# menonsamir/spiral

Hardware: AMD Instinct MI355X
Metric: server ms/query + DB GB/s vs HBM roofline, 2^20 x 256B (lower is better)
Workload: dtype u32 residues, 32x32->64-bit integer MAC (two 28-bit CRT primes)

## Files before the change

### spiral_amd/csrc/host_common.h

```cpp
#pragma once
#include <hip/hip_runtime.h>

#include <algorithm>
#include <atomic>
#include <cstdarg>
#include <cstdio>
#include <cstdlib>
#include <cstring>
#include <string>
#include <vector>

#include "../../include/spiral_gpu.h"
#include "common.h"
#include "kernels.h"
#include "seed_device.h"
#include "transform_jobs.h"

namespace spiral {
namespace host {

extern thread_local std::string g_err;
extern std::atomic<uint64_t> g_pack_lane_batches;
extern std::atomic<uint64_t> g_db_export_ns;

// ... 112 lines not shown
    std::vector<void*> ptrs;
    ~Scratch() {
        for (void* p : ptrs) (void)hipFree(p);
    }
    uint64_t* get(size_t words) {
        void* p = nullptr;
        if (hipMalloc(&p, (words ? words : 1) * sizeof(uint64_t)) != hipSuccess) return nullptr;
        ptrs.push_back(p);
        return (uint64_t*)p;
    }
    uint64_t* upload(const uint64_t* host, size_t words) {
        uint64_t* d = get(words);
        if (d && hipMemcpy(d, host, words * sizeof(uint64_t), hipMemcpyHostToDevice) != hipSuccess) return nullptr;
        return d;
    }
};

inline int current_tables(DeviceTables* t) {
    int dev = 0;
    HIP_OK(hipGetDevice(&dev));
    if (tables_get(dev, t) != 0) return fail("twiddle table setup failed on device %d", dev);
    return 0;
}

struct ExpandWork {
    uint64_t* raw;
    uint64_t* g;
};
inline size_t expand_g_polys(uint32_t g, uint32_t t_exp, uint32_t t_exp_right) {
    size_t half = (size_t)1 << (g ? g - 1 : 0);
    return half * ((size_t)t_exp + 1 + t_exp_right + 1);
}

struct ExpandShard {
    uint32_t rank, g_log, j_log;
};

inline void run_expand(const DeviceTables& tb, uint64_t* cv, uint32_t g, uint32_t t_exp, const uint64_t* w_left, uint32_t t_exp_right,
                const uint64_t* w_right, uint32_t max_bits_right, uint32_t stopround, const ExpandWork& wk, hipStream_t st,
                const uint64_t* query = nullptr,
                uint32_t r_begin = 0, uint32_t r_end = 0xffffffffu,
                const ExpandShard& shard = ExpandShard{},
                uint32_t parity = 3,
                const Lanes& lanes = Lanes{}) {
    auto odd_count = [&](uint32_t r) {
        const uint32_t num_in = 1u << r;
        if (stopround > 0 && r > stopround) return 0u;
        if (stopround > 0 && r == stopround) return std::min(num_in, max_bits_right + 1);
        return num_in;
    };
    for (uint32_t r = r_begin; r < std::min(r_end, g); r++) {
        const uint32_t num_in = 1u << r;
        const uint32_t t = (kN >> r) + 1;
        uint32_t cnt_even = (parity & 1u) ? num_in : 0u, cnt_odd = (parity & 2u) ? odd_count(r) : 0u;
        if (cnt_even + cnt_odd == 0) continue;
        ExpandActive act{};
        if (shard.g_log) {
            if (r > shard.j_log && cnt_even) {
                cnt_even = 1u << shard.j_log;
                act.e_off = (shard.rank & ((1u << (r - shard.j_log)) - 1u)) << shard.j_log;
            }
            if (r >= shard.g_log) {
                const uint32_t G = 1u << shard.g_log;
                cnt_odd = cnt_odd > shard.rank ? (cnt_odd - shard.rank + G - 1u) / G : 0u;
                act.o_stride_m1 = G - 1u;
                act.o_off = shard.rank;
            }
        }
        const uint32_t cnt = cnt_even + cnt_odd;
        InvParams ip{};
        ip.dst = wk.raw;
        ip.src_map = ip.dst_map = identity_map();
        ip.cv = cv;
        ip.neg1 = tb.neg1 + (size_t)r * kN;
        ip.neg1s = tb.neg1s + (size_t)r * kN;
        ip.num_in = num_in;
        ip.cnt_e = cnt_even;
        ip.act = act;
        ip.auto_t = t;
        ip.create_here = r == 0;
        ip.query = query;
        ip.lanes = lanes;
        launch_ntt_inverse_expand(tb, ip, 2 * cnt, st);
        FwdParams fp{};
        fp.src = wk.raw;
        fp.dst = wk.g;
        fp.src_map = fp.dst_map = identity_map();
        fp.n_digits = 1;
        fp.cnt_e = cnt_even;
        fp.t_e = t_exp;
        fp.t_o = t_exp_right;
        fp.lanes = lanes;
        launch_ntt_forward(tb, fp, LD_EXPAND, ST_PK, cnt_even * t_exp + cnt_odd * t_exp_right, st);
        ExpandMacParams mp{};
        mp.cv = cv;
        mp.w_e = w_left + (size_t)r * 2 * t_exp * kN;
        mp.w_o = w_right + (size_t)r * 2 * t_exp_right * kN;
        mp.g = wk.g;
        mp.a1 = wk.raw;
        mp.cnt_e = cnt_even;
        mp.cnt_o = cnt_odd;
        mp.act = act;
        mp.t_e = t_exp;
        mp.t_o = t_exp_right;
        if (r + 1 < g) {
            mp.neg1n = tb.neg1 + (size_t)(r + 1) * kN;
            mp.neg1ns = tb.neg1s + (size_t)(r + 1) * kN;
            mp.next_num_in = 2 * num_in;
            mp.next_cnt_o = odd_count(r + 1);
        }
        mp.lanes = lanes;
        launch_expand_mac_round(mp, st);
    }
}


template <class Launch>
inline int ingest_items(const void* items, uint32_t coeff_bits, uint64_t first, uint64_t lo, uint64_t hi, uint32_t polys_per_item, uint64_t p_db,
                        hipStream_t st, Launch launch) {
    if (!items) return fail("null item stream");
    if (coeff_bits != 64 && (coeff_bits < 1 || coeff_bits > 40)) return fail("coefficient width %u not in 1..40 or 64", coeff_bits);
    if (coeff_bits < 64 && (1ull << coeff_bits) < p_db) return fail("%u-bit coefficients cannot hold values below p_db", coeff_bits);
    if (lo >= hi) return 0;
    const size_t item_bytes = (size_t)polys_per_item * kN * coeff_bits / 8;
    const size_t stage_bytes = options().db_stage_bytes;
    const uint64_t chunk = std::max<uint64_t>(1, std::min<uint64_t>({stage_bytes / item_bytes, (uint64_t)(1u << 16), hi - lo}));
    uint8_t* d_items = nullptr;
    uint32_t* d_err = nullptr;
    HIP_OK(hipMalloc(&d_items, chunk * item_bytes + 16));
    if (hipMalloc(&d_err, sizeof(uint32_t)) != hipSuccess || hipMemsetAsync(d_err, 0, sizeof(uint32_t), st) != hipSuccess) {
        (void)hipFree(d_items);
        return fail("device allocation failed");
    }
    hipError_t e = hipMemsetAsync(d_items + chunk * item_bytes, 0, 16, st);
    for (uint64_t done = lo; done < hi && e == hipSuccess; done += chunk) {
        const uint64_t n = std::min(chunk, hi - done);
        e = hipMemcpyAsync(d_items, (const uint8_t*)items + (size_t)(done - first) * item_bytes, (size_t)n * item_bytes, hipMemcpyHostToDevice, st);
        if (e != hipSuccess) break;
        launch(d_items, d_err, done, n);
        e = hipStreamSynchronize(st);
    }
    uint32_t err = 0;
    if (e == hipSuccess) e = hipMemcpy(&err, d_err, sizeof(err), hipMemcpyDeviceToHost);
    (void)hipFree(d_items);
    (void)hipFree(d_err);
    if (e != hipSuccess) return fail("database ingest failed: %s", hipGetErrorString(e));
    if (err) return fail("a plaintext coefficient is not below p_db (the reference asserts, src/spiral.cpp:1117)");
    return 0;
}

struct UpdateWork {
    DevBuf dev;
    uint8_t* host = nullptr;
    size_t host_bytes = 0;
    hipEvent_t done = nullptr;
    bool pending = false;
    void release() {
        if (pending && done) (void)hipEventSynchronize(done);
        dev.release();
        dev.words = 0;
        if (host) (void)hipHostFree(host);
        host = nullptr;
        host_bytes = 0;
        if (done) (void)hipEventDestroy(done);
        done = nullptr;
        pending = false;
    }
};

inline int check_update_ids(const void* items, const uint64_t* ids, uint64_t n, uint64_t total) {
    if (n == 0) return 0;
    if (!items || !ids) return fail("null argument");
    if (n > (1ull << 24)) return fail("at most 2^24 items per update");
    std::vector<uint64_t> sorted(ids, ids + n);
    std::sort(sorted.begin(), sorted.end());
    if (sorted.back() >= total) return fail("item id %llu outside the database of %llu items", (unsigned long long)sorted.back(), (unsigned long long)total);
    for (uint64_t k = 1; k < n; k++)
        if (sorted[k] == sorted[k - 1]) return fail("item id %llu given twice", (unsigned long long)sorted[k]);
    return 0;
}

inline bool coeffs_below(const uint8_t* item, size_t count, uint32_t coeff_bits, uint64_t p_db) {
    if (coeff_bits == 64) {
        for (size_t i = 0; i < count; i++) {
            uint64_t v;
            memcpy(&v, item + 8 * i, 8);
            if (v >= p_db) return false;
        }
        return true;
    }
    if ((1ull << coeff_bits) <= p_db) return true;
    const uint64_t mask = (1ull << coeff_bits) - 1;
    for (size_t i = 0; i < count; i++) {
        const uint64_t bit = (uint64_t)i * coeff_bits;
// ... 256 lines not shown
```

### spiral_amd/csrc/kernels.h

```cpp
#pragma once
#include <hip/hip_runtime.h>
#include <stdint.h>
#include <stdlib.h>

#include <atomic>

#include "common.h"

namespace spiral {

struct IndexMap {
    uint32_t inner, outer_stride, off;
    __host__ __device__ uint32_t operator()(uint32_t b) const { return (b / inner) * outer_stride + (b % inner) + off; }
};
inline IndexMap identity_map() { return IndexMap{1u, 1u, 0u}; }

#ifdef SPIRAL_TUNING
inline const char* tuning_env(const char* name) { return getenv(name); }
#else
inline const char* tuning_env(const char*) { return nullptr; }
#endif
struct Options {
    int fold_pair = 1, fold_chain = 1, fwd2 = -1;
    uint32_t fold_blocks = 768, sweep_mfma_min = 2, fwd2_min = 8192;
    size_t db_stage_bytes = (size_t)64 << 20;
    int one_image = 1;
    uint32_t pack_item_group = 0;
    uint32_t pack_batch_lanes = 0;
    int pack_pair_blocks = 0;
    int sweep_narrow = 0;
    uint32_t query_batch_chunk = 512;
};
Options& options();

#ifndef SPIRAL_MAX_LANES
#define SPIRAL_MAX_LANES 8
#endif
constexpr uint32_t kMaxLanes = SPIRAL_MAX_LANES;
struct Lanes {
    uint32_t n = 1;
    int64_t off[kMaxLanes] = {};
#ifdef __HIPCC__
    __device__ __forceinline__ int64_t here() const {
        const uint32_t z = blockIdx.z;
        int64_t o = 0;
#pragma unroll
        for (uint32_t q = 1; q < kMaxLanes; q++) o = z == q ? off[q] : o;
        return o;
    }
    __device__ __forceinline__ int64_t at(int64_t stride) const { return (int64_t)blockIdx.z * stride; }
#endif
};
#ifdef __HIPCC__
template <class T>
__device__ __forceinline__ void lane_shift(T*& p, int64_t words) {
    if (p) p = reinterpret_cast<T*>(reinterpret_cast<uintptr_t>(p) + (intptr_t)words * 8);
}
#endif
struct NoLanes {
    uint32_t n = 1;
#ifdef __HIPCC__
    __device__ __forceinline__ int64_t here() const { return 0; }
    __device__ __forceinline__ int64_t at(int64_t) const { return 0; }
#endif
};
struct Slots {
    uint32_t n = 1;
    int64_t stride = 0;
#ifdef __HIPCC__
    __device__ __forceinline__ int64_t here() const { return (int64_t)blockIdx.z * stride; }
    __device__ __forceinline__ int64_t at(int64_t s) const { return (int64_t)blockIdx.z * s; }
#endif
};
template <class P>
inline typename P::NoLanesT no_lanes(const P& p) {
    typename P::NoLanesT q{};
    static_cast<typename P::Core&>(q) = static_cast<const typename P::Core&>(p);
    return q;
}

struct DeviceTables {
    uint4* fwd = nullptr;
    uint4* inv = nullptr;
    uint64_t* neg1 = nullptr;
    uint64_t* neg1s = nullptr;
};
int tables_get(int device, DeviceTables* out);
void tables_host_rows(uint64_t* out8x2048);

constexpr bool lazy_ok(uint32_t terms) { return (unsigned __int128)terms * (2ull * kP - 1ull) * (kP - 1ull) < ((unsigned __int128)1 << 64); }
static_assert(lazy_ok(56) && lazy_ok(2 * 56) && lazy_ok(128) && !lazy_ok(129), "u64 accumulators hold up to 128 lazy products");

enum FwdLoad : uint32_t {
    LD_RAW = 0,
    LD_DIGIT = 1,
    LD_SDIGIT = 2,
    LD_LIMBS = 3,
    LD_DBGEN = 4,
    LD_PDIGIT = 6,
    LD_DBGEN1 = 7,
    LD_SDIFF = 8,
    LD_PDIFF = 9,
    LD_EXPAND = 5,
    LD_WIRE = 10,
};
constexpr uint32_t kWireCoeffBytes = 7;
constexpr uint32_t kWirePolyBytes = kWireCoeffBytes * 2048u;
enum FwdStore : uint32_t {
    ST_PK = 0,
    ST_REF = 1,
    ST_DB = 2,
    ST_DB1 = 3,
};
enum PackMap : uint32_t {
    PM_GSW = 0,
    PM_FOLD = 1,
    PM_PACK = 2,
};
struct FwdParamsCore {
    const uint64_t* src;
    uint64_t* dst;
    IndexMap src_map;
    IndexMap dst_map;
    uint32_t n_digits;
    uint32_t inv_n_digits, inv_te, inv_to;
    uint32_t bits;
    uint32_t ell;
    uint32_t tinv;
    uint32_t lazy_out;
    uint32_t fold_np;
    uint32_t pmode, pk_num_per;
    uint32_t trial;
    uint64_t total_n;
    uint32_t cnt_e, t_e, t_o;
    const uint8_t* items;
    uint32_t coeff_bits;
    uint64_t items_first;
    uint32_t* err;
    uint64_t seed, p_db;
    uint64_t item_base;
    uint32_t num_per, dim0_shard, j0;
};
template <class L>
struct FwdParamsT : FwdParamsCore {
// ... 76 lines not shown
    uint32_t row0;
};
struct KeyBindParams {
    const uint64_t* store;
    uint64_t slot_words;
    uint32_t head;
    uint32_t domain;
    KeyPart part[4];
    uint32_t slot[kMaxLanes];
    Lanes lanes;
};
void launch_key_bind(const KeyBindParams& p, KeyForm form, hipStream_t s);

enum QueryForm : int { QUERY_WIRE = 0, QUERY_SEEDED = 1 };
struct QueryIngestParams {
    const uint8_t* stage;
    uint64_t lane_stride;
    uint32_t head;
    uint64_t* dst;
    uint32_t rows, cols;
    uint32_t domain;
    uint32_t first_dst, first_msg;
    uint32_t msg_polys;
    uint32_t* err;
    uint64_t gen;
    Lanes lanes;
};
void launch_query_ingest(const DeviceTables& t, const QueryIngestParams& p, QueryForm form, uint32_t n_dst, hipStream_t s);

struct MatmulParamsCore {
    const uint64_t* a;
    const uint64_t* b;
    uint64_t* out;
    uint32_t rs, ms, cs;
    uint32_t a_batch, b_batch, out_batch;
};
template <class L>
struct MatmulParamsT : MatmulParamsCore {
    using Core = MatmulParamsCore;
    using NoLanesT = MatmulParamsT<NoLanes>;
    L lanes;
};
using MatmulParams = MatmulParamsT<Lanes>;
void launch_matmul(const MatmulParams& p, uint32_t batch, hipStream_t s);
void launch_fold_mac(const uint64_t* key, const uint64_t* d, uint64_t* out, uint32_t K, uint32_t np, hipStream_t s, uint32_t key_stride = 0,
                     const uint64_t* addend = nullptr, const Lanes& lanes = Lanes{});
void launch_fold_mac_two(const uint64_t* q, const uint64_t* d, uint64_t* out, uint32_t m2, uint32_t ell, uint32_t bits, uint32_t np, hipStream_t s,
                         const Lanes& lanes = Lanes{});
void launch_add(const uint64_t* a, const uint64_t* b, uint64_t* out, uint32_t npolys, hipStream_t s);
void launch_mul_by_const(const uint64_t* single, const uint64_t* a, uint64_t* out, uint32_t npolys, hipStream_t s);
void launch_automorph(const uint64_t* in, uint64_t* out, uint32_t npolys, uint32_t t, hipStream_t s);
void launch_invert(const uint64_t* in, uint64_t* out, uint32_t npolys, hipStream_t s);
void launch_gadget_invert(const uint64_t* in, uint64_t* out, uint32_t mx, uint32_t rdim, uint32_t cols, hipStream_t s);
void launch_rescale(const uint64_t* in, uint64_t* out, uint32_t n, uint64_t inp_mod, uint64_t out_mod, hipStream_t s);
void launch_response_wire(const uint64_t* in, uint64_t* out, uint32_t n0, uint32_t w0, uint32_t n1, uint32_t w1, hipStream_t s, const Lanes& lanes = Lanes{},
                          int64_t in_stride = 0, int64_t out_stride = 0);
void launch_rescale2(const uint64_t* in, uint64_t* out, uint32_t n0, uint32_t n, uint64_t inp_mod, uint64_t out_mod0, uint64_t out_mod1, hipStream_t s,
                     const Lanes& lanes = Lanes{}, int64_t out_stride = 0);
void launch_rescale2_slots(const uint64_t* in, uint64_t* out, uint32_t n0, uint32_t n, uint64_t inp_mod, uint64_t out_mod0, uint64_t out_mod1, const Slots& slots,
                           hipStream_t s);
void launch_response_wire_slots(const uint64_t* in, uint64_t* out, uint32_t n0, uint32_t w0, uint32_t n1, uint32_t w1, const Slots& slots, int64_t out_stride,
                                hipStream_t s);

struct ExpandMacParamsCore {
    uint64_t* cv;
    const uint64_t* w_e;
    const uint64_t* w_o;
    const uint64_t* g;
    const uint64_t* a1;
    uint32_t cnt_e, cnt_o, t_e, t_o;
    ExpandActive act;
    const uint64_t* neg1n;
    const uint64_t* neg1ns;
    uint32_t next_num_in, next_cnt_o;
};
template <class L>
struct ExpandMacParamsT : ExpandMacParamsCore {
    using Core = ExpandMacParamsCore;
    using NoLanesT = ExpandMacParamsT<NoLanes>;
    L lanes;
};
using ExpandMacParams = ExpandMacParamsT<Lanes>;
void launch_expand_mac_round(const ExpandMacParams& p, hipStream_t s);
struct Scal2MatParamsCore {
    const uint64_t* w;
    const uint64_t* g;
    const uint64_t* cv;
    IndexMap cv_pos;
    uint64_t* out;
    uint32_t* qs;
    uint32_t t_conv, count, jm_total, j_base;
};
template <class L>
struct Scal2MatParamsT : Scal2MatParamsCore {
    using Core = Scal2MatParamsCore;
    using NoLanesT = Scal2MatParamsT<NoLanes>;
    L lanes;
};
using Scal2MatParams = Scal2MatParamsT<Lanes>;
void launch_scal2mat(const Scal2MatParams& p, hipStream_t s);
struct GswParamsCore {
    const uint64_t* w;
    const uint64_t* v;
    const uint64_t* chat;
    const uint64_t* cv;
    IndexMap cv_pos;
    uint64_t* gsw;
    uint64_t* key;
    uint32_t t_conv, ell, dims;
};
template <class L>
struct GswParamsT : GswParamsCore {
    using Core = GswParamsCore;
    using NoLanesT = GswParamsT<NoLanes>;
    L lanes;
};
using GswParams = GswParamsT<Lanes>;
void launch_regev_to_gsw(const GswParams& p, hipStream_t s);
void launch_convert_products(const Scal2MatParams& sp, const GswParams& gp, hipStream_t s);
void launch_fold_key_from_reoriented(const uint64_t* q_re, const uint64_t* qneg_re, uint64_t* key, uint32_t m2, hipStream_t s);

void launch_sweep(const uint64_t* db, const uint32_t* qs, uint64_t* acc, uint32_t num_per, uint32_t jm_total, uint32_t g_log, hipStream_t s, uint32_t k_log = 0,
                  int stage = -1);
bool sweep_stages_ok(uint32_t num_per, uint32_t jm_total, uint32_t g_log, uint32_t k_log);
constexpr uint32_t kSweepMaxBatch = 2;
bool sweep_batch_ok(uint32_t num_per, uint32_t jm_total);
void launch_sweep_batch(const uint64_t* db, const uint32_t* const* qs, uint64_t* const* acc, uint32_t n, uint32_t num_per, uint32_t jm_total, uint32_t g_log,
                        hipStream_t s, uint32_t g_extra = 0);
bool sweep_mfma_ok(uint32_t num_per, uint32_t jm_total);
void launch_db_limb_planes(const uint64_t* db_packed_img, uint64_t* db_limbs, uint32_t num_per, uint32_t jm_total, hipStream_t s, uint32_t nz = kN);
void launch_db_limb_unplanes(const uint64_t* db_limbs, uint64_t* db_packed_img, uint32_t num_per, uint32_t jm_total, hipStream_t s, uint32_t nz = kN);
hipError_t launch_sweep_mfma(const uint64_t* db_limbs, const uint32_t* const* qs, uint64_t* const* acc, uint32_t n, uint32_t num_per, uint32_t jm_total, uint32_t g_log,
                             hipStream_t s, uint32_t k_log = 0, uint32_t g_extra = 0);
extern std::atomic<uint64_t> g_mfma_sweeps;
void launch_db_relayout(const uint64_t* db_ref, uint64_t* db_dev, uint32_t num_per, uint32_t dim0, uint32_t j0, uint32_t dim0_shard, uint32_t z0,
                        uint32_t nz, hipStream_t s);
void launch_qs_from_reoriented(const uint64_t* reoriented, uint32_t* qs, uint32_t jm_total, hipStream_t s);
void launch_fill_db_random(uint64_t* db_dev, uint32_t num_per, uint32_t dim0_shard, uint64_t seed, hipStream_t s);
void launch_db_read_item(const uint64_t* db_dev, uint64_t* out_ref, uint32_t num_per, uint32_t dim0_shard, uint32_t j_local, uint32_t ii, hipStream_t s,
                         bool limbs = false);
void launch_db_read_slots(const uint64_t* db_dev, uint64_t* out, uint32_t num_per, uint32_t dim0_shard, uint32_t z0, uint32_t nz, uint32_t ii0, uint32_t n_ii,
                          hipStream_t s, bool limbs = false);
void launch_fill_db1_random(uint64_t* db_dev, uint32_t num_per, uint32_t dim0, uint64_t seed, hipStream_t s);
void launch_gsw_bits_pack(const uint64_t* cv, uint64_t* block, uint32_t rank, uint32_t n_ranks, uint32_t n_bits, hipStream_t s);
void launch_gsw_bits_unpack(uint64_t* cv, const uint64_t* gathered, uint32_t n_ranks, uint32_t n_bits, hipStream_t s);
void launch_gsw_bits_pack_lanes(const uint64_t* cv, uint64_t* block, uint32_t rank, uint32_t n_ranks, uint32_t n_bits, const Lanes& lanes, hipStream_t s);
void launch_gsw_bits_unpack_lanes(uint64_t* cv, const uint64_t* gathered, uint32_t n_ranks, uint32_t n_bits, const Lanes& lanes, hipStream_t s);

__host__ __device__ inline size_t db1_word_index(uint32_t z, uint32_t j, uint32_t ii, uint32_t num_per, uint32_t dim0) {
    const uint32_t w = num_per < 64u ? num_per : 64u, nblk = num_per / w;
    return ((((size_t)z * nblk + ii / w) * (dim0 / 2) + (j >> 1)) * w + ii % w) * 2u + (j & 1u);
}
__host__ __device__ inline bool db1_packed(uint32_t num_per, uint32_t dim0) { return (dim0 & 15u) == 0u && num_per >= 1u && (num_per & (num_per - 1u)) == 0u; }
__host__ __device__ inline size_t db1_device_words(uint32_t num_per, uint32_t dim0) {
    const size_t words = (size_t)kN * dim0 * num_per;
    return db1_packed(num_per, dim0) ? words / 8u * 7u : words;
}
__host__ __device__ inline size_t db1_packed_byte(uint32_t z, uint32_t j, uint32_t ii, uint32_t by, uint32_t num_per, uint32_t dim0) {
    const uint32_t w = num_per < 64u ? num_per : 64u, pz = 64u / w, nblk = num_per / w;
    const uint32_t tile = (z / pz) * nblk + ii / w, lane = (z % pz) * w + ii % w, b = 7u * (j & 15u) + by;
    return ((((size_t)tile * (dim0 >> 4) + (j >> 4)) * 7u + (b >> 4)) * 64u + lane) * 16u + (b & 15u);
}
#ifdef __HIPCC__
__device__ __forceinline__ void db1_put_word(uint64_t* db, uint32_t z, uint32_t j, uint32_t ii, uint32_t num_per, uint32_t dim0, uint64_t v) {
    if (db1_packed(num_per, dim0)) {
        const uint64_t f = (uint64_t)(uint32_t)v | ((uint64_t)(uint32_t)(v >> 32) << 28);
// ... 107 lines not shown
```

### spiral_amd/csrc/poly.hip

```cpp
#include <cstdlib>
#include <type_traits>
#include "common.h"
#include "kernels.h"

namespace spiral {

__device__ __forceinline__ uint32_t shoup32(uint32_t y, uint32_t w, uint32_t ws, uint32_t m) { return w * y - __umulhi(y, ws) * m; }

constexpr uint32_t kTpb = 256;
constexpr uint32_t kBpp = kN / kTpb;

struct Acc2 {
    uint64_t lo = 0, hi = 0;
    __device__ __forceinline__ void mac(uint64_t a, uint64_t b) {
        lo += (uint64_t)lo32(a) * lo32(b);
        hi += (uint64_t)hi32(a) * hi32(b);
    }
    __device__ __forceinline__ uint64_t reduced() const { return pack(mod_p(lo), mod_b(hi)); }
};
__device__ __forceinline__ uint64_t add_pk(uint64_t a, uint64_t b) {
    return pack(csub(lo32(a) + lo32(b), kP), csub(hi32(a) + hi32(b), kB));
}

template <class L>
__global__ __launch_bounds__(kTpb) void matmul_kernel(MatmulParamsT<L> p) {
    const uint32_t z = blockIdx.x * kTpb + threadIdx.x;
    uint32_t rc = blockIdx.y, bt = blockIdx.z;
    if constexpr (!std::is_same<L, NoLanes>::value) {
        const int64_t lane = p.lanes.here();
        lane_shift(p.a, lane);
        lane_shift(p.b, lane);
        lane_shift(p.out, lane);
        bt = blockIdx.y / (p.rs * p.cs);
        rc = blockIdx.y - bt * (p.rs * p.cs);
    }
    const uint32_t r = rc / p.cs, c = rc - r * p.cs;
    const uint64_t* a = p.a + ((size_t)bt * p.a_batch + (size_t)r * p.ms) * kN + z;
    const uint64_t* b = p.b + ((size_t)bt * p.b_batch + c) * kN + z;
    Acc2 acc;
    for (uint32_t m = 0; m < p.ms; m++) acc.mac(a[(size_t)m * kN], b[(size_t)m * p.cs * kN]);
    p.out[((size_t)bt * p.out_batch + rc) * kN + z] = acc.reduced();
}
void launch_matmul(const MatmulParams& p, uint32_t batch, hipStream_t s) {
    if (batch == 0) return;
    if (p.lanes.n > 1)
        hipLaunchKernelGGL(matmul_kernel<Lanes>, dim3(kBpp, p.rs * p.cs * batch, p.lanes.n), dim3(kTpb), 0, s, p);
    else
        hipLaunchKernelGGL(matmul_kernel<NoLanes>, dim3(kBpp, p.rs * p.cs, batch), dim3(kTpb), 0, s, no_lanes(p));
}

struct FoldMacParamsCore {
    const uint64_t* key;
    const uint64_t* d;
    uint64_t* out;
    uint32_t K;
    uint32_t ks;
    const uint64_t* add;
};
template <class L>
struct FoldMacParamsT : FoldMacParamsCore {
    using Core = FoldMacParamsCore;
    using NoLanesT = FoldMacParamsT<NoLanes>;
    L lanes;
};
using FoldMacParams = FoldMacParamsT<Lanes>;
template <uint32_t B, class L>
__global__ __launch_bounds__(kTpb) void fold_mac_kernel(FoldMacParamsT<L> p) {
    __shared__ uint64_t sh[3][64][12 * B];
    const uint32_t zz = threadIdx.x & 63u, kg = threadIdx.x >> 6, z = blockIdx.x * 64u + zz, i0 = blockIdx.y * B;
    {
        const int64_t lane = p.lanes.here();
        lane_shift(p.key, lane);
        lane_shift(p.d, lane);
        lane_shift(p.out, lane);
        lane_shift(p.add, lane);
    }
    const uint64_t* dp = p.d + (size_t)i0 * p.K * 2 * kN + z;
    const uint64_t* kp = p.key + z;
    Acc2 acc[B][3][2];
    if (p.add != nullptr && kg == 0) {
#pragma unroll
        for (uint32_t b = 0; b < B; b++)
#pragma unroll
            for (uint32_t rc = 0; rc < 6; rc++) {
                const uint64_t a = p.add[((size_t)(i0 + b) * 6 + rc) * kN + z];
                acc[b][rc >> 1][rc & 1].lo = lo32(a);
                acc[b][rc >> 1][rc & 1].hi = hi32(a);
            }
    }
    if constexpr (B == 1) {
        constexpr uint32_t U = 12;
        for (uint32_t m0 = kg; m0 < p.K; m0 += 4 * U) {
            uint64_t kv[U][3], dv[U][2];
#pragma unroll
            for (uint32_t u = 0; u < U; u++) {
                const uint32_t mm = min(m0 + 4 * u, p.K - 1);
#pragma unroll
                for (uint32_t r = 0; r < 3; r++) kv[u][r] = kp[((size_t)r * p.ks + mm) * kN];
                dv[u][0] = __builtin_nontemporal_load(&dp[(size_t)mm * 2 * kN]);
                dv[u][1] = __builtin_nontemporal_load(&dp[((size_t)mm * 2 + 1) * kN]);
            }
#pragma unroll
            for (uint32_t u = 0; u < U; u++) {
                if (m0 + 4 * u < p.K) {
#pragma unroll
// ... 204 lines not shown
    const uint32_t ne = mx / rdim, bits = get_bits_per(ne);
    const uint64_t mask = (1ull << bits) - 1;
    const uint64_t v = in[((size_t)j * cols + c) * kN + z];
    for (uint32_t k = 0; k < ne; k++) {
        uint32_t sh = k * bits;
        out[((size_t)(j + k * rdim) * cols + c) * kN + z] = sh >= 64 ? 0ull : ((v >> sh) & mask);
    }
}
void launch_gadget_invert(const uint64_t* in, uint64_t* out, uint32_t mx, uint32_t rdim, uint32_t cols, hipStream_t s) {
    hipLaunchKernelGGL(gadget_invert_kernel, dim3(kBpp, rdim * cols), dim3(kTpb), 0, s, in, out, mx, rdim, cols);
}

__global__ __launch_bounds__(kTpb) void rescale_kernel(const uint64_t* in, uint64_t* out, uint32_t n, uint64_t inp_mod, uint64_t out_mod) {
    const uint32_t i = blockIdx.x * kTpb + threadIdx.x;
    if (i < n) out[i] = rescale_dev(in[i] % kQ, inp_mod, out_mod);
}
template <class L>
__global__ __launch_bounds__(kTpb) void rescale2_kernel(const uint64_t* in, uint64_t* out, uint32_t n0, uint32_t n, uint64_t inp_mod, uint64_t out_mod0,
                                                        uint64_t out_mod1, L lanes, int64_t out_stride) {
    const uint32_t i = blockIdx.x * kTpb + threadIdx.x;
    lane_shift(in, lanes.here());
    lane_shift(out, out_stride ? lanes.at(out_stride) : lanes.here());
    if (i < n) out[i] = rescale_dev(in[i] % kQ, inp_mod, i < n0 ? out_mod0 : out_mod1);
}
template <class L>
__global__ __launch_bounds__(kTpb) void response_wire_kernel(const uint64_t* in, uint64_t* out, uint32_t n0, uint32_t w0, uint32_t n1, uint32_t w1, L lanes,
                                                             int64_t in_stride, int64_t out_stride) {
    const uint32_t k = blockIdx.x * kTpb + threadIdx.x;
    lane_shift(in, in_stride ? lanes.at(in_stride) : lanes.here());
    lane_shift(out, lanes.at(out_stride));
    const uint32_t words0 = n0 / 64u * w0, words1 = n1 / 64u * w1;
    if (k >= words0 + words1) return;
    const bool second = k >= words0;
    const uint32_t w = second ? w1 : w0;
    const uint64_t bit0 = (uint64_t)(second ? k - words0 : k) * 64u;
    const uint64_t* v = in + (second ? n0 : 0);
    const uint32_t nv = second ? n1 : n0;
    const uint64_t mask = (1ull << w) - 1;
    uint64_t word = 0;
    for (uint32_t i = (uint32_t)(bit0 / w); i < nv && (uint64_t)i * w < bit0 + 64; i++) {
        const uint64_t x = v[i] & mask;
        const int64_t sh = (int64_t)((uint64_t)i * w) - (int64_t)bit0;
        word |= sh >= 0 ? x << sh : x >> (-sh);
    }
    out[k] = word;
}
void launch_response_wire(const uint64_t* in, uint64_t* out, uint32_t n0, uint32_t w0, uint32_t n1, uint32_t w1, hipStream_t s, const Lanes& lanes,
                          int64_t in_stride, int64_t out_stride) {
    const uint32_t words = n0 / 64u * w0 + n1 / 64u * w1;
    if (lanes.n > 1)
        hipLaunchKernelGGL(response_wire_kernel<Lanes>, dim3((words + kTpb - 1) / kTpb, 1, lanes.n), dim3(kTpb), 0, s, in, out, n0, w0, n1, w1, lanes, in_stride,
                           out_stride);
    else
        hipLaunchKernelGGL(response_wire_kernel<NoLanes>, dim3((words + kTpb - 1) / kTpb), dim3(kTpb), 0, s, in, out, n0, w0, n1, w1, NoLanes{}, (int64_t)0,
                           (int64_t)0);
}
void launch_rescale2(const uint64_t* in, uint64_t* out, uint32_t n0, uint32_t n, uint64_t inp_mod, uint64_t out_mod0, uint64_t out_mod1, hipStream_t s,
                     const Lanes& lanes, int64_t out_stride) {
    if (n == 0) return;
    if (lanes.n > 1)
        hipLaunchKernelGGL(rescale2_kernel<Lanes>, dim3((n + kTpb - 1) / kTpb, 1, lanes.n), dim3(kTpb), 0, s, in, out, n0, n, inp_mod, out_mod0, out_mod1, lanes,
                           out_stride);
    else
        hipLaunchKernelGGL(rescale2_kernel<NoLanes>, dim3((n + kTpb - 1) / kTpb, 1, 1), dim3(kTpb), 0, s, in, out, n0, n, inp_mod, out_mod0, out_mod1, NoLanes{},
                           (int64_t)0);
}
void launch_rescale2_slots(const uint64_t* in, uint64_t* out, uint32_t n0, uint32_t n, uint64_t inp_mod, uint64_t out_mod0, uint64_t out_mod1, const Slots& slots,
                           hipStream_t s) {
    if (n && slots.n)
        hipLaunchKernelGGL(rescale2_kernel<Slots>, dim3((n + kTpb - 1) / kTpb, 1, slots.n), dim3(kTpb), 0, s, in, out, n0, n, inp_mod, out_mod0, out_mod1, slots,
                           (int64_t)slots.stride);
}
void launch_response_wire_slots(const uint64_t* in, uint64_t* out, uint32_t n0, uint32_t w0, uint32_t n1, uint32_t w1, const Slots& slots, int64_t out_stride,
                                hipStream_t s) {
    const uint32_t words = n0 / 64u * w0 + n1 / 64u * w1;
    if (slots.n)
        hipLaunchKernelGGL(response_wire_kernel<Slots>, dim3((words + kTpb - 1) / kTpb, 1, slots.n), dim3(kTpb), 0, s, in, out, n0, w0, n1, w1, slots,
                           (int64_t)slots.stride, out_stride);
}
void launch_rescale(const uint64_t* in, uint64_t* out, uint32_t n, uint64_t inp_mod, uint64_t out_mod, hipStream_t s) {
    if (n) hipLaunchKernelGGL(rescale_kernel, dim3((n + kTpb - 1) / kTpb), dim3(kTpb), 0, s, in, out, n, inp_mod, out_mod);
}

template <class P>
__device__ __forceinline__ void expand_mac_lane(P& p) {
    const int64_t lane = p.lanes.here();
    lane_shift(p.cv, lane);
    lane_shift(p.w_e, lane);
    lane_shift(p.w_o, lane);
    lane_shift(p.g, lane);
    lane_shift(p.a1, lane);
}
template <class L>
__global__ __launch_bounds__(kTpb) void expand_mac_round_kernel(ExpandMacParamsT<L> p) {
    __shared__ uint64_t sh[3][64][4];
    expand_mac_lane(p);
    const uint32_t zz = threadIdx.x & 63u, kg = threadIdx.x >> 6, z = blockIdx.x * 64u + zz, a = blockIdx.y;
    const bool odd = a >= p.cnt_e;
    const uint32_t tdim = odd ? p.t_o : p.t_e;
    const uint32_t i = p.act.index(a, p.cnt_e);
    const size_t gbase = odd ? (size_t)p.cnt_e * p.t_e + (size_t)(a - p.cnt_e) * p.t_o : (size_t)a * p.t_e;
    const uint64_t* w = (odd ? p.w_o : p.w_e) + z;
    const uint64_t* gp = p.g + gbase * kN + z;
    const bool make_next = kg == 0 && p.neg1n != nullptr && (!odd || (i >> 1) + (p.next_num_in >> 1) < p.next_cnt_o);
    uint64_t nw = 0, nws = 0;
    if (make_next) {
        nw = p.neg1n[z];
        nws = p.neg1ns[z];
    }
    uint64_t* c = p.cv + (size_t)i * 2 * kN + z;
    uint64_t old0 = 0, old1 = 0, a1v = 0;
    if (kg == 0) {
        old0 = c[0];
        old1 = c[kN];
        a1v = p.a1[((size_t)a * 2u + 1u) * kN + z];
    }
    Acc2 acc0, acc1;
#pragma unroll 14
    for (uint32_t k = kg; k < tdim; k += 4) {
#ifndef MAC_PLAIN_LOADS
        const uint64_t gv = __builtin_nontemporal_load(&gp[(size_t)k * kN]);
#else
        const uint64_t gv = gp[(size_t)k * kN];
#endif
        acc0.mac(w[(size_t)k * kN], gv);
        acc1.mac(w[(size_t)(tdim + k) * kN], gv);
    }
    if (kg > 0) {
        sh[kg - 1][zz][0] = acc0.lo;
        sh[kg - 1][zz][1] = acc0.hi;
        sh[kg - 1][zz][2] = acc1.lo;
        sh[kg - 1][zz][3] = acc1.hi;
    }
    __syncthreads();
    if (kg == 0) {
#pragma unroll
        for (int q = 0; q < 3; q++) {
            acc0.lo += sh[q][zz][0];
            acc0.hi += sh[q][zz][1];
            acc1.lo += sh[q][zz][2];
            acc1.hi += sh[q][zz][3];
        }
        const uint64_t c0 = add_pk(old0, acc0.reduced());
        const uint64_t c1 = add_pk(add_pk(old1, acc1.reduced()), a1v);
        c[0] = c0;
        c[kN] = c1;
        if (make_next) {
            uint64_t* n = p.cv + (size_t)(i + p.next_num_in) * 2 * kN + z;
            n[0] = pack(csub(shoup32(lo32(c0), lo32(nw), lo32(nws), kP), kP), csub(shoup32(hi32(c0), hi32(nw), hi32(nws), kB), kB));
            n[kN] = pack(csub(shoup32(lo32(c1), lo32(nw), lo32(nws), kP), kP), csub(shoup32(hi32(c1), hi32(nw), hi32(nws), kB), kB));
        }
    }
}
typedef unsigned long long u64x2_t __attribute__((ext_vector_type(2)));
template <class L>
__global__ __launch_bounds__(kTpb) void expand_mac_round_wide_kernel(ExpandMacParamsT<L> p) {
    __shared__ uint64_t sh[3][64][8];
    expand_mac_lane(p);
    const uint32_t zz = threadIdx.x & 63u, kg = threadIdx.x >> 6, z = (blockIdx.x * 64u + zz) * 2u, a = blockIdx.y;
    const bool odd = a >= p.cnt_e;
    const uint32_t tdim = odd ? p.t_o : p.t_e;
    const uint32_t i = p.act.index(a, p.cnt_e);
    const size_t gbase = odd ? (size_t)p.cnt_e * p.t_e + (size_t)(a - p.cnt_e) * p.t_o : (size_t)a * p.t_e;
    const uint64_t* w = (odd ? p.w_o : p.w_e) + z;
    const uint64_t* gp = p.g + gbase * kN + z;
    const bool make_next = kg == 0 && p.neg1n != nullptr && (!odd || (i >> 1) + (p.next_num_in >> 1) < p.next_cnt_o);
    u64x2_t nw = {0, 0}, nws = {0, 0};
    if (make_next) {
        nw = *reinterpret_cast<const u64x2_t*>(p.neg1n + z);
        nws = *reinterpret_cast<const u64x2_t*>(p.neg1ns + z);
    }
    uint64_t* c = p.cv + (size_t)i * 2 * kN + z;
    u64x2_t old0 = {0, 0}, old1 = {0, 0}, a1v = {0, 0};
    if (kg == 0) {
        old0 = *reinterpret_cast<const u64x2_t*>(c);
// ... 561 lines not shown
```

### spiral_amd/csrc/primitives.cpp

```cpp
#include "server_state.h"

thread_local std::string spiral::host::g_err;
std::atomic<uint64_t> spiral::host::g_pack_lane_batches{0};
std::atomic<uint64_t> spiral::g_mfma_sweeps{0};
std::atomic<uint64_t> spiral::host::g_db_export_ns{0};

spiral::Options& spiral::options() {
    static Options o = [] {
        Options v;
        if (const char* e = getenv("SPIRAL_FOLD_PAIR")) v.fold_pair = atoi(e) != 0;
        if (const char* e = getenv("SPIRAL_SWEEP_MFMA")) v.sweep_mfma_min = (uint32_t)strtoul(e, nullptr, 10);
        if (const char* e = getenv("SPIRAL_DB_STAGE_BYTES")) v.db_stage_bytes = (size_t)strtoull(e, nullptr, 10);
        return v;
    }();
    return o;
}

namespace {
size_t base_message_bytes(const spiral_gpu_params* p, MessageLayout (*layout)(const spiral_gpu_params&, const spiral_gpu_shape&), Form form) {
    spiral_gpu_shape s;
    return shape_of(p, &s) ? 0 : message_bytes(layout(*p, s), form);
}
}

extern "C" {

int spiral_gpu_abi_version(void) { return SPIRAL_GPU_ABI_VERSION; }

int spiral_gpu_set_option(const char* name, int64_t value) {
    if (!name) return fail("null option name");
    Options& o = options();
    const std::string n = name;
    if (n == "fold_pair") o.fold_pair = value != 0;
    else if (n == "fold_chain") o.fold_chain = value != 0;
    else if (n == "fold_blocks" && value >= 0) o.fold_blocks = (uint32_t)value;
    else if (n == "sweep_mfma_min" && value >= 0) o.sweep_mfma_min = (uint32_t)value;
    else if (n == "one_image") o.one_image = value != 0;
    else if (n == "fwd2" && value >= -1 && value <= 1) o.fwd2 = (int)value;
    else if (n == "fwd2_min" && value >= 0) o.fwd2_min = (uint32_t)value;
    else if (n == "db_stage_bytes" && value > 0) o.db_stage_bytes = (size_t)value;
    else if (n == "pack_item_group" && value >= 0 && value <= 0xFFFFFFFFll) o.pack_item_group = (uint32_t)value;
    else if (n == "pack_batch_lanes" && value >= 0 && value <= (int64_t)kMaxLanes) o.pack_batch_lanes = (uint32_t)value;
    else if (n == "pack_pair_blocks" && (value == 0 || value == 1)) o.pack_pair_blocks = (int)value;
    else if (n == "sweep_narrow" && (value == 0 || value == 1)) o.sweep_narrow = (int)value;
    else if (n == "query_batch_chunk" && value >= 1 && value <= 0xFFFFFFFFll) o.query_batch_chunk = (uint32_t)value;
    else return fail("unknown option '%s' or value %lld out of range", name, (long long)value);
    return 0;
}
int spiral_gpu_get_option(const char* name, int64_t* value) {
    if (!name || !value) return fail("null argument");
    const Options& o = options();
    const std::string n = name;
    if (n == "fold_pair") *value = o.fold_pair;
    else if (n == "fold_chain") *value = o.fold_chain;
    else if (n == "fold_blocks") *value = o.fold_blocks;
    else if (n == "sweep_mfma_min") *value = o.sweep_mfma_min;
    else if (n == "one_image") *value = o.one_image;
    else if (n == "fwd2") *value = o.fwd2;
    else if (n == "fwd2_min") *value = o.fwd2_min;
    else if (n == "db_stage_bytes") *value = (int64_t)o.db_stage_bytes;
    else if (n == "pack_item_group") *value = o.pack_item_group;
    else if (n == "pack_batch_lanes") *value = o.pack_batch_lanes;
    else if (n == "pack_pair_blocks") *value = o.pack_pair_blocks;
    else if (n == "sweep_narrow") *value = o.sweep_narrow;
    else if (n == "query_batch_chunk") *value = o.query_batch_chunk;
    else if (n == "graph_captures") *value = (int64_t)g_captures.load();
    else if (n == "pack_lane_batches") *value = (int64_t)g_pack_lane_batches.load();
    else if (n == "key_binds") *value = (int64_t)g_key_binds.load();
    else if (n == "db_export_ns") *value = (int64_t)g_db_export_ns.load();
    else if (n == "mfma_sweeps") *value = (int64_t)g_mfma_sweeps.load(std::memory_order_relaxed);
    else return fail("unknown option '%s'", name);
    return 0;
}
const char* spiral_gpu_last_error(void) { return g_err.c_str(); }
int spiral_gpu_device_count(void) {
    int n = 0;
    if (hipGetDeviceCount(&n) != hipSuccess) return 0;
    return n;
}
int spiral_gpu_get_shape(const spiral_gpu_params* p, spiral_gpu_shape* out) { return shape_of(p, out); }
int spiral_gpu_has_limb_form(const spiral_gpu_params* p, uint32_t j_begin, uint32_t j_end) {
    if (!p) return fail("null argument");
    spiral_gpu_shape s;
    spiral_gpu_params q = *p;
    q.direct_upload = 1;
    if (shape_of(&q, &s)) return -1;
    if (j_end == 0 && j_begin == 0) j_end = s.dim0;
    if (j_begin >= j_end || j_end > s.dim0) return fail("bad first-dimension shard [%u, %u) of %u", j_begin, j_end, s.dim0);
    return DbLayout::base(s.num_per, j_end - j_begin).limbs_ok() ? 1 : 0;
}
int spiral_gpu_get_tables(uint64_t* out) {
    if (!out) return fail("null argument");
    tables_host_rows(out);
    return 0;
}

int spiral_gpu_ntt_forward(uint64_t* operand, size_t npolys) {
    DeviceTables tb;
    if (current_tables(&tb)) return -1;
    Scratch sc;
    uint64_t* d = sc.upload(operand, npolys * kRefNtt);
    if (!d) return fail("device allocation/upload failed");
    FwdParams fp{};
    fp.src = d;
    fp.dst = d;
    fp.src_map = fp.dst_map = identity_map();
    fp.n_digits = 1;
    launch_ntt_forward(tb, fp, LD_LIMBS, ST_REF, (uint32_t)npolys, 0);
    HIP_OK(hipMemcpy(operand, d, npolys * kRefNtt * sizeof(uint64_t), hipMemcpyDeviceToHost));
    return 0;
}

int spiral_gpu_ntt_inverse(uint64_t* operand, size_t npolys) {
    DeviceTables tb;
    if (current_tables(&tb)) return -1;
    Scratch sc;
    uint64_t* d = sc.upload(operand, npolys * kRefNtt);
    if (!d) return fail("device allocation/upload failed");
    InvParams ip{};
    ip.src = d;
    ip.dst = d;
    ip.src_map = ip.dst_map = identity_map();
    ip.src_ref = 1;
    ip.pre_reduce = 1;
    launch_ntt_inverse(tb, ip, IST_LIMBS, (uint32_t)npolys, 0);
    HIP_OK(hipMemcpy(operand, d, npolys * kRefNtt * sizeof(uint64_t), hipMemcpyDeviceToHost));
    return 0;
}

int spiral_gpu_to_ntt(uint64_t* out, const uint64_t* in, size_t npolys, int reduce) {
    DeviceTables tb;
    if (current_tables(&tb)) return -1;
    Scratch sc;
    uint64_t* d_in = sc.upload(in, npolys * kN);
    uint64_t* d_out = sc.get(npolys * kRefNtt);
    if (!d_in || !d_out) return fail("device allocation/upload failed");
    if (reduce) {
        launch_job(tb, raw_job(d_in, d_out, (uint32_t)npolys, ST_REF), 0);
    } else {
        uint64_t* d_pk = sc.get(npolys * kN);
        if (!d_pk) return fail("device allocation failed");
        launch_job(tb, raw32_job(d_in, d_pk, (uint32_t)npolys), 0);
// ... 369 lines not shown
```

Before: 0.7365.

## Fuse query-expansion forward NTT with the key-switch MAC into one kernel

```diff
diff --git a/spiral_amd/csrc/expand_fused.hip b/spiral_amd/csrc/expand_fused.hip
--- /dev/null
+++ b/spiral_amd/csrc/expand_fused.hip
@@ -0,0 +1,199 @@
+#include <algorithm>
+
+#include "digits_device.h"
+#include "kernels.h"
+#include "mac_device.h"
+#include "ntt_device.h"
+
+namespace spiral {
+
+struct ExpandFinish {
+    uint64_t* c;
+    uint64_t* nx;
+};
+template <class P>
+__device__ __forceinline__ ExpandFinish expand_finish_of(const P& p, uint32_t a, bool odd) {
+    const uint32_t i = p.act.index(a, p.cnt_e);
+    const bool make_next = p.neg1n != nullptr && (!odd || (i >> 1) + (p.next_num_in >> 1) < p.next_cnt_o);
+    uint64_t* c = p.cv + (size_t)i * 2 * kN;
+    return ExpandFinish{c, make_next ? p.cv + (size_t)(i + p.next_num_in) * 2 * kN : nullptr};
+}
+
+template <class L>
+__global__ __launch_bounds__(256, 3) void expand_fused_kernel(Tables t, ExpandMacParamsT<L> p, uint64_t* part, ExpandChunks ch) {
+    __shared__ uint64_t sh[kLdsWords];
+    __shared__ uint64_t keep[kN];
+    const uint32_t tid = threadIdx.x;
+    uint32_t b = blockIdx.x, lane = blockIdx.z;
+    if (ch.lane_log) {
+        lane = blockIdx.x & ((1u << ch.lane_log) - 1u);
+        b = (blockIdx.x >> ch.lane_log) + (gridDim.x >> ch.lane_log) * blockIdx.z;
+    }
+    if (b >= ch.nblocks) return;
+    {
+        const int64_t off = p.lanes.of(lane);
+        lane_shift(p.cv, off);
+        lane_shift(p.w_e, off);
+        lane_shift(p.w_o, off);
+        lane_shift(p.a1, off);
+        lane_shift(part, off);
+    }
+    const uint32_t je = p.cnt_e * ch.ch_e;
+    const bool odd = b >= je;
+    const uint32_t bb = odd ? b - je : b, chunks = odd ? ch.ch_o : ch.ch_e, dpc = odd ? ch.dpc_o : ch.dpc_e, tdim = odd ? p.t_o : p.t_e;
+    const uint32_t as = bb / chunks, c = bb - as * chunks, a = odd ? as + p.cnt_e : as;
+    const uint32_t k0 = c * dpc, k1 = min(k0 + dpc, tdim);
+    const uint64_t* w = odd ? p.w_o : p.w_e;
+    const uint64_t* src = p.a1 + (size_t)a * 2u * kN;
+    {
+        uint64_t raw[8];
+#pragma unroll
+        for (int r = 0; r < 8; r++) raw[r] = src[ix_a(tid, r)];
+#pragma unroll
+        for (int r = 0; r < 8; r++) keep[ix_a(tid, r)] = raw[r];
+    }
+    const uint32_t bits = get_bits_per(tdim);
+    const uint64_t mask = (1ull << bits) - 1;
+    auto digits = [&](uint32_t k, uint32_t* lo, uint32_t* hi) {
+        uint64_t raw[8];
+#pragma unroll
+        for (int r = 0; r < 8; r++) raw[r] = keep[ix_a(tid, r)];
+        if (bits <= kSmallDigitBits) {
+            udigits8(raw, k, bits, lo);
+#pragma unroll
+            for (int r = 0; r < 8; r++) hi[r] = lo[r];
+        } else {
+#pragma unroll
+            for (int r = 0; r < 8; r++) {
+                const uint32_t d = (uint32_t)digit_of(raw[r], k, bits, mask);
+                lo[r] = digit_residue<false>(d, kP);
+                hi[r] = digit_residue<false>(d, kB);
+            }
+        }
+    };
+    Acc2 acc[2][8];
+    auto mac = [&](uint32_t k, const uint32_t* lo, const uint32_t* hi) {
+        uint64_t w0[8], w1[8];
+        pk_load8(w + (size_t)k * kN, tid, w0);
+        pk_load8(w + (size_t)(tdim + k) * kN, tid, w1);
+#pragma unroll
+        for (int r = 0; r < 8; r++) {
+            const uint64_t d = pack(lo[r], hi[r]);
+            acc[0][r].mac(w0[r], d);
+            acc[1][r].mac(w1[r], d);
+        }
+    };
+    for (uint32_t k = k0; k < k1; k++) {
+        uint32_t lo[8], hi[8];
+        digits(k, lo, hi);
+        if (k > k0) __syncthreads();
+        ntt_forward_block<false>(lo, hi, sh, t.fwd, tid);
+        mac(k, lo, hi);
+    }
+    uint64_t s0[8], s1[8];
+#pragma unroll
+    for (int r = 0; r < 8; r++) {
+        s0[r] = acc[0][r].reduced();
+        s1[r] = acc[1][r].reduced();
+    }
+    if (chunks > 1) {
+        const uint32_t slot = odd ? (ch.ch_e > 1 ? je : 0u) + bb : b;
+        pk_store8(part + (size_t)slot * 2u * kN, tid, s0);
+        pk_store8(part + ((size_t)slot * 2u + 1u) * kN, tid, s1);
+        return;
+    }
+    const ExpandFinish f = expand_finish_of(p, a, odd);
+    uint64_t old0[8], old1[8], a1v[8];
+    pk_load8(f.c, tid, old0);
+    pk_load8(f.c + kN, tid, old1);
+    pk_load8(src + kN, tid, a1v);
+#pragma unroll
+    for (int r = 0; r < 8; r++) {
+        s0[r] = add_pk(old0[r], s0[r]);
+        s1[r] = add_pk(add_pk(old1[r], s1[r]), a1v[r]);
+    }
+    pk_store8(f.c, tid, s0);
+    pk_store8(f.c + kN, tid, s1);
+    if (f.nx) {
+        uint64_t nw[8], nws[8];
+        pk_load8(p.neg1n, tid, nw);
+        pk_load8(p.neg1ns, tid, nws);
+#pragma unroll
+        for (int r = 0; r < 8; r++) {
+            s0[r] = neg1_times(s0[r], nw[r], nws[r]);
+            s1[r] = neg1_times(s1[r], nw[r], nws[r]);
+        }
+        pk_store8(f.nx, tid, s0);
+        pk_store8(f.nx + kN, tid, s1);
+    }
+}
+
+typedef unsigned long long fz_u64x2 __attribute__((ext_vector_type(2)));
+template <class L>
+__global__ __launch_bounds__(256) void expand_fused_finish_kernel(ExpandMacParamsT<L> p, const uint64_t* part, ExpandChunks ch, uint32_t a_first) {
+    expand_mac_lane(p);
+    lane_shift(part, p.lanes.here());
+    const uint32_t z = (blockIdx.x * 256u + threadIdx.x) * 2u, a = a_first + blockIdx.y;
+    const bool odd = a >= p.cnt_e;
+    const uint32_t chunks = odd ? ch.ch_o : ch.ch_e;
+    const uint32_t slot0 = odd ? (ch.ch_e > 1 ? p.cnt_e * ch.ch_e : 0u) + (a - p.cnt_e) * chunks : a * chunks;
+    const ExpandFinish f = expand_finish_of(p, a, odd);
+    auto ld = [&](const uint64_t* q) { return *reinterpret_cast<const fz_u64x2*>(q + z); };
+    const fz_u64x2 old0 = ld(f.c), old1 = ld(f.c + kN), a1v = ld(p.a1 + ((size_t)a * 2u + 1u) * kN);
+    fz_u64x2 nw = {0, 0}, nws = {0, 0};
+    if (f.nx) {
+        nw = ld(p.neg1n);
+        nws = ld(p.neg1ns);
+    }
+    const uint64_t* pp = part + (size_t)slot0 * 2u * kN;
+    fz_u64x2 s0 = ld(pp), s1 = ld(pp + kN);
+    for (uint32_t c = 1; c < chunks; c++) {
+        const fz_u64x2 x0 = ld(pp + (size_t)c * 2u * kN), x1 = ld(pp + ((size_t)c * 2u + 1u) * kN);
+        s0 = fz_u64x2{add_pk(s0.x, x0.x), add_pk(s0.y, x0.y)};
+        s1 = fz_u64x2{add_pk(s1.x, x1.x), add_pk(s1.y, x1.y)};
+    }
+    const fz_u64x2 c0 = {add_pk(old0.x, s0.x), add_pk(old0.y, s0.y)};
+    const fz_u64x2 c1 = {add_pk(add_pk(old1.x, s1.x), a1v.x), add_pk(add_pk(old1.y, s1.y), a1v.y)};
+    *reinterpret_cast<fz_u64x2*>(f.c + z) = c0;
+    *reinterpret_cast<fz_u64x2*>(f.c + kN + z) = c1;
+    if (f.nx) {
+        *reinterpret_cast<fz_u64x2*>(f.nx + z) = fz_u64x2{neg1_times(c0.x, nw.x, nws.x), neg1_times(c0.y, nw.y, nws.y)};
+        *reinterpret_cast<fz_u64x2*>(f.nx + kN + z) = fz_u64x2{neg1_times(c1.x, nw.x, nws.x), neg1_times(c1.y, nw.y, nws.y)};
+    }
+}
+
+void launch_expand_fused(const DeviceTables& t, const ExpandMacParams& p, uint64_t* part, hipStream_t s) {
+    if (p.cnt_e + p.cnt_o == 0) return;
+    constexpr uint32_t kMaxDpc = 14, kBlocks = 768, kMinDpc = 3;
+    ExpandChunks ch{};
+    auto chunks_of = [](uint32_t tdim, uint32_t dpc) { return (tdim + dpc - 1u) / dpc; };
+    ch.dpc_e = std::max(p.t_e, 1u);
+    ch.dpc_o = std::max(p.t_o, 1u);
+    auto blocks = [&] { return (uint64_t)(p.cnt_e * chunks_of(p.t_e, ch.dpc_e) + p.cnt_o * chunks_of(p.t_o, ch.dpc_o)) * p.lanes.n; };
+    auto split = [&](uint32_t& dpc, uint32_t cnt) {
+        while (cnt && dpc > kMinDpc && (dpc > kMaxDpc || blocks() < kBlocks)) dpc = std::max((dpc + 1u) / 2u, kMinDpc);
+    };
+    split(ch.dpc_o, p.cnt_o);
+    split(ch.dpc_e, p.cnt_e);
+    ch.ch_e = chunks_of(p.t_e, ch.dpc_e);
+    ch.ch_o = chunks_of(p.t_o, ch.dpc_o);
+    const uint32_t nblocks = p.cnt_e * ch.ch_e + p.cnt_o * ch.ch_o;
+    ch.nblocks = nblocks;
+    uint32_t gx = nblocks;
+    if (p.lanes.n == 2 || p.lanes.n == 4 || p.lanes.n == 8) {
+        ch.lane_log = p.lanes.n == 2 ? 1u : p.lanes.n == 4 ? 2u : 3u;
+        gx = (nblocks + 7u) & ~7u;
+    }
+    const uint32_t a_first = ch.ch_e > 1 ? 0u : p.cnt_e, n_fin = (ch.ch_e > 1 ? p.cnt_e : 0u) + (ch.ch_o > 1 ? p.cnt_o : 0u);
+    const Tables tb{t.fwd, t.inv};
+    if (p.lanes.n > 1) {
+        hipLaunchKernelGGL(expand_fused_kernel<Lanes>, dim3(gx, 1, p.lanes.n), dim3(256), 0, s, tb, p, part, ch);
+        if (n_fin) hipLaunchKernelGGL(expand_fused_finish_kernel<Lanes>, dim3(kN / 512, n_fin, p.lanes.n), dim3(256), 0, s, p, (const uint64_t*)part, ch, a_first);
+    } else {
+        const auto q = no_lanes(p);
+        hipLaunchKernelGGL(expand_fused_kernel<NoLanes>, dim3(nblocks, 1, 1), dim3(256), 0, s, tb, q, part, ch);
+        if (n_fin) hipLaunchKernelGGL(expand_fused_finish_kernel<NoLanes>, dim3(kN / 512, n_fin, 1), dim3(256), 0, s, q, (const uint64_t*)part, ch, a_first);
+    }
+}
+
+}
diff --git a/spiral_amd/csrc/host_common.h b/spiral_amd/csrc/host_common.h
--- a/spiral_amd/csrc/host_common.h
+++ b/spiral_amd/csrc/host_common.h
@@ -218,16 +218,6 @@
         ip.query = query;
         ip.lanes = lanes;
         launch_ntt_inverse_expand(tb, ip, 2 * cnt, st);
-        FwdParams fp{};
-        fp.src = wk.raw;
-        fp.dst = wk.g;
-        fp.src_map = fp.dst_map = identity_map();
-        fp.n_digits = 1;
-        fp.cnt_e = cnt_even;
-        fp.t_e = t_exp;
-        fp.t_o = t_exp_right;
-        fp.lanes = lanes;
-        launch_ntt_forward(tb, fp, LD_EXPAND, ST_PK, cnt_even * t_exp + cnt_odd * t_exp_right, st);
         ExpandMacParams mp{};
         mp.cv = cv;
         mp.w_e = w_left + (size_t)r * 2 * t_exp * kN;
@@ -246,6 +236,22 @@
             mp.next_cnt_o = odd_count(r + 1);
         }
         mp.lanes = lanes;
+        const uint64_t transforms = (uint64_t)(cnt_even * t_exp + cnt_odd * t_exp_right) * lanes.n;
+        const int fuse_opt = options().expand_fuse;
+        if (fuse_opt >= 0 ? fuse_opt != 0 : transforms >= options().expand_fuse_min) {
+            launch_expand_fused(tb, mp, wk.g, st);
+            continue;
+        }
+        FwdParams fp{};
+        fp.src = wk.raw;
+        fp.dst = wk.g;
+        fp.src_map = fp.dst_map = identity_map();
+        fp.n_digits = 1;
+        fp.cnt_e = cnt_even;
+        fp.t_e = t_exp;
+        fp.t_o = t_exp_right;
+        fp.lanes = lanes;
+        launch_ntt_forward(tb, fp, LD_EXPAND, ST_PK, cnt_even * t_exp + cnt_odd * t_exp_right, st);
         launch_expand_mac_round(mp, st);
     }
 }
diff --git a/spiral_amd/csrc/kernels.h b/spiral_amd/csrc/kernels.h
--- a/spiral_amd/csrc/kernels.h
+++ b/spiral_amd/csrc/kernels.h
@@ -21,8 +21,8 @@
 inline const char* tuning_env(const char*) { return nullptr; }
 #endif
 struct Options {
-    int fold_pair = 1, fold_chain = 1, fwd2 = -1;
-    uint32_t fold_blocks = 768, sweep_mfma_min = 2, fwd2_min = 8192;
+    int fold_pair = 1, fold_chain = 1, fwd2 = -1, expand_fuse = -1;
+    uint32_t fold_blocks = 768, sweep_mfma_min = 2, fwd2_min = 8192, expand_fuse_min = 8192;
     size_t db_stage_bytes = (size_t)64 << 20;
     int one_image = 1;
     uint32_t pack_item_group = 0;
@@ -41,13 +41,13 @@
     uint32_t n = 1;
     int64_t off[kMaxLanes] = {};
 #ifdef __HIPCC__
-    __device__ __forceinline__ int64_t here() const {
-        const uint32_t z = blockIdx.z;
+    __device__ __forceinline__ int64_t of(uint32_t z) const {
         int64_t o = 0;
 #pragma unroll
         for (uint32_t q = 1; q < kMaxLanes; q++) o = z == q ? off[q] : o;
         return o;
     }
+    __device__ __forceinline__ int64_t here() const { return of(blockIdx.z); }
     __device__ __forceinline__ int64_t at(int64_t stride) const { return (int64_t)blockIdx.z * stride; }
 #endif
 };
@@ -60,6 +60,7 @@
 struct NoLanes {
     uint32_t n = 1;
 #ifdef __HIPCC__
+    __device__ __forceinline__ int64_t of(uint32_t) const { return 0; }
     __device__ __forceinline__ int64_t here() const { return 0; }
     __device__ __forceinline__ int64_t at(int64_t) const { return 0; }
 #endif
@@ -302,6 +303,12 @@
 };
 using ExpandMacParams = ExpandMacParamsT<Lanes>;
 void launch_expand_mac_round(const ExpandMacParams& p, hipStream_t s);
+struct ExpandChunks {
+    uint32_t dpc_e, ch_e, dpc_o, ch_o;
+    uint32_t nblocks;
+    uint32_t lane_log;
+};
+void launch_expand_fused(const DeviceTables& t, const ExpandMacParams& p, uint64_t* part, hipStream_t s);
 struct Scal2MatParamsCore {
     const uint64_t* w;
     const uint64_t* g;
diff --git a/spiral_amd/csrc/mac_device.h b/spiral_amd/csrc/mac_device.h
--- /dev/null
+++ b/spiral_amd/csrc/mac_device.h
@@ -0,0 +1,34 @@
+#pragma once
+#include "common.h"
+#include "kernels.h"
+
+namespace spiral {
+
+__device__ __forceinline__ uint32_t shoup32(uint32_t y, uint32_t w, uint32_t ws, uint32_t m) { return w * y - __umulhi(y, ws) * m; }
+
+struct Acc2 {
+    uint64_t lo = 0, hi = 0;
+    __device__ __forceinline__ void mac(uint64_t a, uint64_t b) {
+        lo += (uint64_t)lo32(a) * lo32(b);
+        hi += (uint64_t)hi32(a) * hi32(b);
+    }
+    __device__ __forceinline__ uint64_t reduced() const { return pack(mod_p(lo), mod_b(hi)); }
+};
+__device__ __forceinline__ uint64_t add_pk(uint64_t a, uint64_t b) {
+    return pack(csub(lo32(a) + lo32(b), kP), csub(hi32(a) + hi32(b), kB));
+}
+__device__ __forceinline__ uint64_t neg1_times(uint64_t c, uint64_t w, uint64_t ws) {
+    return pack(csub(shoup32(lo32(c), lo32(w), lo32(ws), kP), kP), csub(shoup32(hi32(c), hi32(w), hi32(ws), kB), kB));
+}
+
+template <class P>
+__device__ __forceinline__ void expand_mac_lane(P& p) {
+    const int64_t lane = p.lanes.here();
+    lane_shift(p.cv, lane);
+    lane_shift(p.w_e, lane);
+    lane_shift(p.w_o, lane);
+    lane_shift(p.g, lane);
+    lane_shift(p.a1, lane);
+}
+
+}
diff --git a/spiral_amd/csrc/poly.hip b/spiral_amd/csrc/poly.hip
--- a/spiral_amd/csrc/poly.hip
+++ b/spiral_amd/csrc/poly.hip
@@ -2,25 +2,12 @@
 #include <type_traits>
 #include "common.h"
 #include "kernels.h"
+#include "mac_device.h"
 
 namespace spiral {
-
-__device__ __forceinline__ uint32_t shoup32(uint32_t y, uint32_t w, uint32_t ws, uint32_t m) { return w * y - __umulhi(y, ws) * m; }
 
 constexpr uint32_t kTpb = 256;
 constexpr uint32_t kBpp = kN / kTpb;
-
-struct Acc2 {
-    uint64_t lo = 0, hi = 0;
-    __device__ __forceinline__ void mac(uint64_t a, uint64_t b) {
-        lo += (uint64_t)lo32(a) * lo32(b);
-        hi += (uint64_t)hi32(a) * hi32(b);
-    }
-    __device__ __forceinline__ uint64_t reduced() const { return pack(mod_p(lo), mod_b(hi)); }
-};
-__device__ __forceinline__ uint64_t add_pk(uint64_t a, uint64_t b) {
-    return pack(csub(lo32(a) + lo32(b), kP), csub(hi32(a) + hi32(b), kB));
-}
 
 template <class L>
 __global__ __launch_bounds__(kTpb) void matmul_kernel(MatmulParamsT<L> p) {
@@ -391,15 +378,6 @@
     if (n) hipLaunchKernelGGL(rescale_kernel, dim3((n + kTpb - 1) / kTpb), dim3(kTpb), 0, s, in, out, n, inp_mod, out_mod);
 }
 
-template <class P>
-__device__ __forceinline__ void expand_mac_lane(P& p) {
-    const int64_t lane = p.lanes.here();
-    lane_shift(p.cv, lane);
-    lane_shift(p.w_e, lane);
-    lane_shift(p.w_o, lane);
-    lane_shift(p.g, lane);
-    lane_shift(p.a1, lane);
-}
 template <class L>
 __global__ __launch_bounds__(kTpb) void expand_mac_round_kernel(ExpandMacParamsT<L> p) {
     __shared__ uint64_t sh[3][64][4];
diff --git a/spiral_amd/csrc/primitives.cpp b/spiral_amd/csrc/primitives.cpp
--- a/spiral_amd/csrc/primitives.cpp
+++ b/spiral_amd/csrc/primitives.cpp
@@ -38,6 +38,8 @@
     else if (n == "one_image") o.one_image = value != 0;
     else if (n == "fwd2" && value >= -1 && value <= 1) o.fwd2 = (int)value;
     else if (n == "fwd2_min" && value >= 0) o.fwd2_min = (uint32_t)value;
+    else if (n == "expand_fuse" && value >= -1 && value <= 1) o.expand_fuse = (int)value;
+    else if (n == "expand_fuse_min" && value >= 0 && value <= 0xFFFFFFFFll) o.expand_fuse_min = (uint32_t)value;
     else if (n == "db_stage_bytes" && value > 0) o.db_stage_bytes = (size_t)value;
     else if (n == "pack_item_group" && value >= 0 && value <= 0xFFFFFFFFll) o.pack_item_group = (uint32_t)value;
     else if (n == "pack_batch_lanes" && value >= 0 && value <= (int64_t)kMaxLanes) o.pack_batch_lanes = (uint32_t)value;
@@ -58,6 +60,8 @@
     else if (n == "one_image") *value = o.one_image;
     else if (n == "fwd2") *value = o.fwd2;
     else if (n == "fwd2_min") *value = o.fwd2_min;
+    else if (n == "expand_fuse") *value = o.expand_fuse;
+    else if (n == "expand_fuse_min") *value = o.expand_fuse_min;
     else if (n == "db_stage_bytes") *value = (int64_t)o.db_stage_bytes;
     else if (n == "pack_item_group") *value = o.pack_item_group;
     else if (n == "pack_batch_lanes") *value = o.pack_batch_lanes;
```

After: 0.7503. 1.9% more time.
